# jake3991/sonar-SLAM

Hardware: AMD Instinct MI355X
Metric: keyframes/sec (CFAR+ICP) on 512x1024 sonar, 5k-pt pairs (higher is better)
Workload: dtype u8 (CFAR, integer-exact) + f32/f64-accumulate (ICP); 1 GPU; BASELINE configs[1]: 4096 keyframes/step/GPU = 1024x512 SOCA-CFAR(Ntc40,Ngc10)+gate65 -> remap+nonzero+px2m -> downsample 0.5 -> remove_outlier 1.0/5 -> 5000x5000-pt ICP (p2plane30); batch_per_gpu=4096, distinct_frames=256, screened_out_pings=0, icp_mode=p2plane30, parallelism=job farm x1, icp_prep_stream=side, batches_in_flight=1, icp_converged_jobs=4096, max_points_per_frame=17494, points_capacity=32768, full=False

## Files before the change

sonar_slam_amd/csrc/sfe_icp_sweep.h:

```cpp
#pragma once
#include "sfe_icp_common.h"

#include <algorithm>
#include <cstdlib>
#include <cstring>
#include <map>
#include <type_traits>
#include <utility>

#define SW_TCAP 8192
#define SW_NS_MAX 64
#define SW_PAD (SW_NS_MAX + 4)
#define SW_GRID_MAX 8192
#define SW_T0_NT 64
#define SW_T0_TCAP 512
#define SW_T0_GRID 512
#define SW_T1_NT 256
#define SW_T1_TCAP 2048
#define SW_T1_GRID 2048
#define SW_MG_MAX 16
#define SW_MG_WORDS 272

struct StripTab {
    int ns, len;
// ... 250 lines not shown
#else
#define SW_STAMP(k)                                                                              \
    do {                                                                                         \
        if (PROF && threadIdx.x == 0 && blockIdx.x == 0 && it == SW_STAMP_ITER)                  \
            prof[85 + (k)] = clock64();                                                          \
    } while (0)
#endif

#define SW_WATCH(cnt, bound, code)                                                               \
    if (++(cnt) > (bound)) {                                                                     \
        if (dbg)                                                                                 \
            atomicMax(dbg + (code), (int)blockIdx.x + 1);                                        \
        break;                                                                                   \
    }
#define SW_NQ 8
#define SW_NONE (-1)
#define SW_INEXACT_OF(bpos) (-2 - (bpos))
#define SW_OWN_DONE 0x80000000u
#define SW_TIED 0x40000000u
#define SW_PARTIAL 0x20000000u
#define SW_QMASK 0x1FFFFFFFu
#define SW_REC_MIN_ITER 12

struct SweepQ {
    int4 *st;
    float *d2;
    int *pos;
    int *wl[2];
    int *mid;
    int *lng;
    int *order;
    int *slot_of;
    unsigned *rec;
    float2 *ssrc;
    const int *perm;
};


struct SweepLaunchArgs {
    sfe_ctx *ctx;
    const sfe_icp_params *p;
    const SweepJob *d_jobs;
    const float2 *d_src;
    const float *d_guess9;
    const float2 *d_stgt;
    const int *d_perm;
    const float2 *d_snrm;
    const float *d_mean;
    const StripTab *d_tab;
    const int *d_grid;
    int4 *d_qst;
    int *d_qwl;
    float2 *d_qssrc;
    float *d_nn_d2;
    int *d_nn_pos;
    float *d_T9;
    int32_t *d_status, *d_iters;
    long long *d_prof;
    int *d_dbg;
    int sw_budget, sw_budget_a, sw_cache, sw_cache2;
    float sw_m, sw_kappa;
    unsigned long long *d_sync;
    sfe_icp_outliers ox;
};

template <int NT, bool PROF, bool REC>
constexpr size_t sweep_ctl_bytes()
{
    return (sizeof(SweepShared<NT, PROF, REC>) + 15) & ~(size_t)15;
}

template <int NT, int MINW, bool LDS_TGT, bool LDS_Q, bool PROF, bool REC, bool MULTI>
int sweep_launch_loop(const SweepLaunchArgs &a, int n, const int *d_ids, size_t body, int t_cap, int q_cap);

template <int NT, int TCAP, int GM, bool GTAIL = false, int KMF = 0>
int sweep_launch_prep(sfe_ctx *ctx, hipStream_t ps, const sfe_icp_params *p, int n, const SweepPrep *d_preps, const int *d_pids,
// ... 17 lines not shown
```

sonar_slam_amd/csrc/sfe_icp_sweep.hip:

```cpp
#include "sfe_icp_sweep.h"

#include <vector>

int sfe_icp_sweep_launch(sfe_ctx *ctx, const sfe_icp_params *p, const IcpCall &call, const float *d_src, const float *d_tgt,
                         const int32_t *jobs4, const float *d_guess9, int n_jobs, float *d_T9, int32_t *d_status,
                         int32_t *d_iters)
{
    std::vector<SweepPrep> preps;
    std::vector<SweepJob> jobs;
    jobs.reserve((size_t)n_jobs);
    std::vector<int> ids_tiny, ids_t0, ids_t1, ids_q, ids_lds, ids_glb, ids_multi, split_first;
    std::vector<int> pids[3];
    std::vector<int> prep_tier;
    std::vector<char> prep_need;
    std::vector<int> pids_nrm;
    std::map<std::pair<int, int>, int> seen;
    long long toff = 0, qoff = 0, koff = 0, goff = 0;
    const sfe_tuning &tu = ctx->tune;
    const bool multi_on = tu.sw_multi && !(ctx->icp_variant & 16) && !call.unsplit;
    const int strip_pts = tu.sw_strip_pts;
    const long long tiny_pairs = (p->use_diff_checker || p->max_iter < SW_REC_MIN_ITER) ? SW_TINY_PAIRS_SHORT : SW_TINY_PAIRS_LONG;
    auto is_tiny = [&](int n_src, int n_tgt) {
        return tu.sw_tiny && n_src <= SW_TINY_MAX && n_tgt <= SW_TINY_MAX && (long long)n_src * n_tgt <= tiny_pairs;
    };
// ... 120 lines not shown
        for (int r : ids_q)
            route[jobs[(size_t)r].out] = SFE_ICP_ROUTE_LDS;
        std::sort(ids_lds.begin(), ids_lds.end());
        ids_q.clear();
    }
    const int n_prep = (int)preps.size(), n_rec = (int)jobs.size();
    const int n_tiny = (int)ids_tiny.size();
    const int n_t0 = (int)ids_t0.size(), n_t1 = (int)ids_t1.size(), n_q = (int)ids_q.size(), n_lds = (int)ids_lds.size(),
              n_glb = (int)ids_glb.size(), n_multi = (int)ids_multi.size(), n_split = (int)split_first.size();
    const size_t o_jobs = (sizeof(SweepPrep) * (size_t)n_prep + 15) & ~(size_t)15;
    const size_t o_ids = (o_jobs + sizeof(SweepJob) * (size_t)n_rec + 15) & ~(size_t)15;
    const size_t o_split = o_ids + sizeof(int) * (size_t)n_rec;
    const size_t o_pids = o_split + sizeof(int) * (size_t)n_split;
    const size_t o_pnrm = o_pids + sizeof(int) * (size_t)n_prep;
    const size_t tab_bytes = o_pnrm + sizeof(int) * pids_nrm.size();
    const bool side = (ctx->icp_variant & 8) != 0;
    const SfeIcpGenPlan gen = sfe_icp_gen_begin(ctx->icp_gens, side, n_split > 0);
    if (gen.sync_first) {
        SFE_HIP(ctx, hipStreamSynchronize(ctx->stream2));
        SFE_HIP(ctx, hipStreamSynchronize(ctx->stream));
    }
    enum { G_TABLES, G_STGT, G_PERM, G_SNRM, G_MEAN, G_GKEYS, G_TAB, G_GRID, G_N };
    static const int gen_slot[2][G_N] = {{12, 14, 15, 16, 17, 24, 23, 38}, {72, 73, 74, 75, 76, 77, 78, 79}};
    static_assert(SFE_NSCRATCH == 80, "generation 1 takes the last eight slots");
    const int *gs = gen_slot[gen.g];
    char *d_tables = (char *)sfe_scratch(ctx, gs[G_TABLES], tab_bytes);
    float2 *d_stgt = (float2 *)sfe_scratch(ctx, gs[G_STGT], sizeof(float2) * (size_t)toff);
    int *d_perm = (int *)sfe_scratch(ctx, gs[G_PERM], sizeof(int) * (size_t)toff);
    float2 *d_snrm = p->minimizer == 1 ? (float2 *)sfe_scratch(ctx, gs[G_SNRM], sizeof(float2) * (size_t)toff) : nullptr;
    float *d_mean = (float *)sfe_scratch(ctx, gs[G_MEAN], sizeof(float) * 2 * (size_t)n_prep);
    unsigned long long *d_gkeys =
        (unsigned long long *)sfe_scratch(ctx, gs[G_GKEYS], sizeof(unsigned long long) * (size_t)std::max(koff, 1LL));
    int4 *d_qst = (int4 *)sfe_scratch(ctx, 19, sizeof(int4) * (size_t)qoff);
    int *d_qwl = (int *)sfe_scratch(ctx, 21, sizeof(int) * 7 * (size_t)qoff);
    float2 *d_qssrc = (float2 *)sfe_scratch(ctx, 30, sizeof(float2) * (size_t)qoff);
    StripTab *d_tab = (StripTab *)sfe_scratch(ctx, gs[G_TAB], sizeof(StripTab) * (size_t)n_prep);
    int *d_grid = (int *)sfe_scratch(ctx, gs[G_GRID], sizeof(int) * (size_t)goff);
    float *d_nn_d2 = (float *)sfe_scratch(ctx, 5, sizeof(float) * (size_t)qoff);
    int *d_nn_pos = (int *)sfe_scratch(ctx, 6, sizeof(int) * (size_t)qoff);
    if (!d_tables || !d_stgt || !d_perm || (p->minimizer == 1 && !d_snrm) || !d_mean || !d_gkeys || !d_qst || !d_qwl || !d_qssrc || !d_tab || !d_grid ||
        !d_nn_d2 || !d_nn_pos)
        return SFE_ERR_HIP;
    float2 *d_gsrc = nullptr;
    unsigned long long *d_sync = nullptr;
    const size_t sync_bytes = sizeof(unsigned long long) * 2 * SW_MG_MAX * SW_MG_WORDS * (size_t)n_sync;
    if (n_split) {
        d_gsrc = (float2 *)sfe_scratch(ctx, 46, sizeof(float2) * (size_t)qoff);
        d_sync = (unsigned long long *)sfe_scratch(ctx, 45, sync_bytes);
        if (!d_gsrc || !d_sync)
            return SFE_ERR_HIP;
    }
    SweepPrep *d_preps = (SweepPrep *)d_tables;
    SweepJob *d_jobs = (SweepJob *)(d_tables + o_jobs);
    int *d_ids = (int *)(d_tables + o_ids);
    int *d_split = (int *)(d_tables + o_split);
    int *d_pids = (int *)(d_tables + o_pids);
    hipStream_t ps = side ? ctx->stream2 : ctx->stream;
    for (int g = 0; g < 2; ++g)
        if (gen.wait[g])
            SFE_HIP(ctx, hipStreamWaitEvent(ps, ctx->ev_loop[g], 0));
    if (gen.wait_begin)
        SFE_HIP(ctx, hipStreamWaitEvent(ps, ctx->ev_loop_begin, 0));
    {
// ... 85 lines not shown
            return SFE_ERR_HIP;
        SFE_HIP(ctx, hipMemsetAsync(d_dbg, 0, sizeof(int) * 8, ctx->stream));
    }
    long long *d_prof = ctx->icp_prof ? (long long *)sfe_scratch(ctx, 20, sizeof(long long) * SFE_ICP_PROF_N) : nullptr;
    if (ctx->icp_prof && !d_prof)
        return SFE_ERR_HIP;
    if (d_prof)
        SFE_HIP(ctx, hipMemsetAsync(d_prof, 0, sizeof(long long) * SFE_ICP_PROF_N, ctx->stream));
    SFE_HIP(ctx, hipEventRecord(ctx->ev_loop_begin, ctx->stream));
    SweepLaunchArgs a;
    a.ctx = ctx;
    a.p = p;
    a.d_jobs = d_jobs;
    a.d_src = (const float2 *)d_src;
    a.d_guess9 = d_guess9;
    a.d_stgt = d_stgt;
    a.d_perm = d_perm;
    a.d_snrm = d_snrm;
    a.d_mean = d_mean;
    a.d_tab = d_tab;
    a.d_grid = d_grid;
    a.d_qst = d_qst;
    a.d_qwl = d_qwl;
    a.d_qssrc = d_qssrc;
    a.d_nn_d2 = d_nn_d2;
    a.d_nn_pos = d_nn_pos;
    a.d_T9 = d_T9;
    a.d_status = d_status;
    a.d_iters = d_iters;
    a.d_prof = d_prof;
    a.d_dbg = d_dbg;
    a.sw_budget = tu.sw_budget;
    a.sw_budget_a = tu.sw_budget_a;
    a.sw_cache = sw_cache;
    a.sw_cache2 = tu.sw_union_iters | (tu.sw_union_max << 8);
    a.sw_m = 0.01f * (float)tu.sw_recm;
    a.sw_kappa = tu.sw_reck;
    a.d_sync = d_sync;
    a.ox = call.ox;
    const bool rec_build = (sw_cache & 16) != 0 && p->max_iter >= SW_REC_MIN_ITER && !p->use_diff_checker;
    int rc = 0;
    const int *ids = d_ids;
    if (n_tiny) {
        if ((rc = sweep_launch_tiny(ctx, p, n_tiny, d_jobs, ids, d_preps, (const float2 *)d_src, (const float2 *)d_tgt, d_guess9,
                                    (const int *)d_perm, (const float2 *)d_snrm, (const float *)d_mean, (const StripTab *)d_tab, d_T9,
                                    d_status, d_iters, tiny_tmax, tiny_smax, call.ox)))
            return rc;
// ... 111 lines not shown
```

sonar_slam_amd/csrc/sfe_icp_sweep_loop.hip:

```cpp
#include "sfe_icp_sweep.h"


template <class TV>
__device__ __forceinline__ int sweep_resolve_tie(const TV &T, const StripTab &tab, const SweepQ &Q,
                                                 float px, float py, float best)
{
    int bo = 0x7FFFFFFF, bp = 0;
    const int ns = tab.ns, so = strip_of(py, tab.ylo, tab.inv_g, ns);
    int s_up = so, s_dn = so - 1;
    for (int guard = 0; guard < 2 * SW_NS_MAX + 2; ++guard) {
        const int s = next_strip(tab, ns, so, s_up, s_dn, py, best);
        if (s < 0)
            break;
        const int lo = strip_lower_bound_lane(T, tab.sbeg[s], tab.sbeg[s + 1] - 1, px);
        for (int dir = 0; dir < 2; ++dir) {
            for (int j = dir ? lo : lo - 1;; j += dir ? 1 : -1) {
                const float2 t = T[j];
                const float dx = f_add(px, -t.x), e = f_mul(dx, dx);
                if (!(e <= best))
                    break;
                const float dy = f_add(py, -t.y);
                if (f_add(e, f_mul(dy, dy)) == best) {
                    const int o = Q.perm[j - 1];
                    if (o < bo) {
                        bo = o;
                        bp = j;
                    }
                }
            }
        }
    }
    return bp;
}

template <int NT, int MINW, bool LDS_TGT, bool LDS_Q, bool PROF, bool REC, bool MULTI, bool OX>
__global__ __launch_bounds__(NT, MINW) __attribute__((amdgpu_waves_per_eu(MINW, MINW))) void icp_sweep_kernel(
    sfe_icp_params P, const SweepJob *__restrict__ jobs, const int *__restrict__ job_ids, const float2 *__restrict__ src_all,
    const float *__restrict__ guess_all, const float2 *__restrict__ stgt_all, const int *__restrict__ perm_all,
    const float2 *__restrict__ snrm_all, const float *__restrict__ mean_all, const StripTab *__restrict__ tab_all,
    const int *__restrict__ grid_all, int4 *__restrict__ q_st_all, int *__restrict__ q_wl_all, float2 *__restrict__ q_ssrc_all,
    float *__restrict__ nn_d2_all,
    int *__restrict__ nn_pos_all, float *__restrict__ T_out, int *__restrict__ status_out,
    int *__restrict__ iters_out, long long *prof, int *dbg, int sw_budget, int sw_budget_a, int sw_cache, int t_cap, int q_cap, int sort_chunk, float sw_m, float sw_kappa,
    unsigned long long *__restrict__ sync_all, int sw_cache2, sfe_icp_outliers O_arg)
{
    const sfe_icp_outliers O = OX ? O_arg : sfe_icp_outliers{};

    static_assert(LDS_TGT || !LDS_Q, "LDS_Q needs the LDS-resident target layout");
    static_assert(!MULTI || !PROF, "the profile build runs whole jobs");
    static_assert(!MULTI || !REC, "split jobs run without clearance records");
    extern __shared__ __attribute__((aligned(16))) char smem_raw[];
    using Shared = SweepShared<NT, PROF, REC>;
    Shared &S = *reinterpret_cast<Shared *>(smem_raw);

    const int jb = __builtin_amdgcn_readfirstlane(job_ids[blockIdx.x]);
    SweepJob J = jobs[jb];
    J.src_start = __builtin_amdgcn_readfirstlane(J.src_start);
    J.n_src = __builtin_amdgcn_readfirstlane(J.n_src);
    J.n_tgt = __builtin_amdgcn_readfirstlane(J.n_tgt);
    J.prep = __builtin_amdgcn_readfirstlane(J.prep);
    J.out = __builtin_amdgcn_readfirstlane(J.out);
    J.grp = __builtin_amdgcn_readfirstlane(J.grp);
    J.ngrp = __builtin_amdgcn_readfirstlane(J.ngrp);
    J.sync = __builtin_amdgcn_readfirstlane(J.sync);
// ... 13 lines not shown
    float *l_d2 = reinterpret_cast<float *>(lds_tgt + t_cap);
    short *l_pos = reinterpret_cast<short *>(l_d2 + q_cap);
    auto Pz = [&](int i) -> int {
        if constexpr (LDS_Q)
            return (int)l_pos[i];
        else
            return Q.pos[i];
    };
    auto Dz = [&](int i) -> float {
        if constexpr (LDS_Q)
            return l_d2[i];
        else
            return Q.d2[i];
    };
    auto setQ = [&](int i, float d, int pz) {
        if constexpr (LDS_Q) {
            l_d2[i] = d;
            l_pos[i] = (short)pz;
        } else {
            Q.d2[i] = d;
            Q.pos[i] = pz;
        }
    };
    Q.wl[0] = q_wl_all + 7 * J.q_off;
    Q.wl[1] = Q.wl[0] + ns;
    Q.mid = Q.wl[1] + ns;
    Q.lng = Q.mid + ns;
    Q.order = Q.lng + ns;
    Q.slot_of = Q.order + ns;
    Q.rec = reinterpret_cast<unsigned *>(Q.slot_of + ns);
    Q.ssrc = q_ssrc_all + J.q_off;
    Q.perm = perm_all + J.tgt_off;
    const float *guess = guess_all + 9 * (size_t)J.out;
    const int tid = threadIdx.x, lane = threadIdx.x & 63;
    const float mx = sw_uniform(mean_all[2 * J.prep]), my = sw_uniform(mean_all[2 * J.prep + 1]);

    if (PROF && tid == 0) {
        for (int i = 0; i < 16; ++i)
            S.prof[i] = 0;
        for (int i = 0; i < 64; ++i)
            S.prof_it[i] = 0;
        S.prof_t = clock64();
    }
    unsigned long long c_eval = 0, c_coop = 0, c_wit = 0, c_lb = 0;
    if (tid == 0) {
        S.rmax_bits = 0u;
        S.xabort = 0;
    }
    {
        const int *tsrc = reinterpret_cast<const int *>(tab_all + J.prep);
        int *tdst = reinterpret_cast<int *>(&S.tab);
        for (int i = tid; i < (int)(sizeof(StripTab) / sizeof(int)); i += NT)
            tdst[i] = tsrc[i];
    }

    float T0[9];
    {
        const float Tinv[9] = {1, 0, -mx, 0, 1, -my, 0, 0, 1};
        float g[9];
#pragma unroll
        for (int i = 0; i < 9; ++i)
            g[i] = guess[i];
        mat3_mul(Tinv, g, T0);
#pragma unroll
        for (int i = 0; i < 9; ++i)
            T0[i] = sw_uniform(T0[i]);
    }
    __syncthreads();

    typedef __attribute__((address_space(1))) unsigned long long gu64;
    unsigned xepoch = 0;
    gu64 *xsync = MULTI ? (gu64 *)(sync_all + (size_t)J.sync * (size_t)(2 * SW_MG_MAX * SW_MG_WORDS)) : nullptr;
    auto xpoll = [&](gu64 *g, unsigned epoch) -> unsigned {
        unsigned long long x = __hip_atomic_load(g, __ATOMIC_RELAXED, __HIP_MEMORY_SCOPE_AGENT);
        if ((unsigned)(x >> 32) != epoch) {
            const unsigned long long t0 = wall_clock64();
            while (true) {
                __builtin_amdgcn_s_sleep(8);
                x = __hip_atomic_load(g, __ATOMIC_RELAXED, __HIP_MEMORY_SCOPE_AGENT);
                if ((unsigned)(x >> 32) == epoch)
                    break;
                if (wall_clock64() - t0 > 50000000ull) {
                    S.xabort = 1;
                    break;
                }
            }
        }
        return (unsigned)x;
    };
    auto xbail = [&]() {
// ... 29 lines not shown
        if (tid < 20)
            __hip_atomic_store(bank + J.grp * SW_MG_WORDS + tid,
                               ((unsigned long long)xepoch << 32) | reinterpret_cast<const unsigned *>(S.acc)[tid],
                               __ATOMIC_RELAXED, __HIP_MEMORY_SCOPE_AGENT);
        double tot = 0.0;
        if (tid < 10) {
            for (int w = 0; w < J.ngrp; ++w) {
                const unsigned lo = xpoll(bank + w * SW_MG_WORDS + 2 * tid, xepoch);
                const unsigned hi = xpoll(bank + w * SW_MG_WORDS + 2 * tid + 1, xepoch);
                tot += __hiloint2double((int)hi, (int)lo);
            }
        }
        __syncthreads();
        if (tid < 10)
            S.acc[tid] = tot;
        __syncthreads();
        if (S.xabort)
            xbail();
    };
    const int *__restrict__ grid = (grid_all != nullptr && (sw_cache & 4) != 0)
                                       ? grid_all + 64 * (size_t)__builtin_amdgcn_readfirstlane(S.tab.grid_off64) : nullptr;

    {
        unsigned long long *skeys = reinterpret_cast<unsigned long long *>(lds_tgt);
        float rloc = 0.0f;
        int *scnt = reinterpret_cast<int *>(S.hist);
        auto qpos = [&](int q) {
            const float2 sp = src[q];
            return make_float2(affine1(T0[0], T0[1], T0[2], sp.x, sp.y), affine1(T0[3], T0[4], T0[5], sp.x, sp.y));
        };
        for (int c0 = 0; c0 < ns; c0 += sort_chunk) {
            const int n = min(sort_chunk, ns - c0);
            unsigned n2 = 2;
            while (n2 < (unsigned)n)
                n2 <<= 1;
            if (tid < SW_NS_MAX)
                scnt[tid] = 0;
            __syncthreads();
            for (unsigned i = tid; i < (unsigned)n; i += NT) {
                const float2 r = qpos(c0 + i);
                atomicAdd(&scnt[strip_of(r.y, S.tab.ylo, S.tab.inv_g, S.tab.ns)], 1);
                const float rr = sqrtf(f_add(f_mul(r.x, r.x), f_mul(r.y, r.y)));
                rloc = (rr > rloc || rr != rr) ? rr : rloc;
            }
            __syncthreads();
            strip_sort_lds<NT>(skeys, (unsigned)n, n2, scnt, reinterpret_cast<int *>(S.hist0), [&](unsigned i) {
                const float2 r = qpos(c0 + i);
                return SW_KEY(strip_of(r.y, S.tab.ylo, S.tab.inv_g, S.tab.ns), mono_key(r.x), c0 + i);
            });
            for (int i = tid; i < n; i += NT) {
                const int q = SW_KEY_ID(skeys[i]);
                Q.order[c0 + i] = q;
                Q.ssrc[c0 + i] = src[q];
                Q.slot_of[q] = c0 + i;
                Q.rec[c0 + i] = 0u;
            }
            __syncthreads();
        }
        atomicMax(&S.rmax_bits, __float_as_uint(rloc));
    }
    if (LDS_TGT) {
        for (int i = tid; i < nt + SW_PAD; i += NT)
            lds_tgt[i] = stgt[i];
    }
    if (tid == 0) {
        S.chk_n[0] = 1;
        S.chk_n[1] = 0;
        S.chk_n[2] = 0;
        const float I[9] = {1, 0, 0, 0, 1, 0, 0, 0, 1};
        for (int i = 0; i < 9; ++i)
            S.Ti[i] = I[i];
        S.flag_iterate = 1;
        S.flag_status = SFE_ICP_OK;
        S.hist_c[0] = 1.0f;
        S.hist_s[0] = 0.0f;
        S.hist_x[0] = 0.0f;
        S.hist_y[0] = 0.0f;
    }
// ... 12 lines not shown
    if constexpr (OX) {
        if (O.use_median && O.median_factor < 1.0f)
            Cmax = sw_uniform(r2_match);
    }
    float Cinit;
    {
        const float h = 8.0f * tab.ext_x / (float)nt;
        Cinit = h * h;
        if (!(Cinit > 1e-30f) || !(Cinit < Cmax))
            Cinit = Cmax;
        Cinit = sw_uniform(Cinit);
    }
    float Cnext = sw_uniform(P.use_trimmed_filter ? Cinit : Cmax);
    if constexpr (OX) {
        if (O.use_median)
            Cnext = sw_uniform(Cinit);
    }
    SW_PROF(0);

    const int sw_rtrips = (sw_cache >> 8) & 255;
    const bool sw_jump = (sw_cache & 2) != 0;
    const float sw_margin = sw_uniform(1.0f + 0.01f * (float)((sw_cache >> 16) & 255));
    int wd_outer = 0;
    auto xform = [&](const float (&Ti)[9], float2 sp) {
        const float rx = affine1(T0[0], T0[1], T0[2], sp.x, sp.y);
        const float ry = affine1(T0[3], T0[4], T0[5], sp.x, sp.y);
        return make_float2(affine1(Ti[0], Ti[1], Ti[2], rx, ry), affine1(Ti[3], Ti[4], Ti[5], rx, ry));
    };
    bool use_cache = false;
    const bool sw_rec = REC && (sw_cache & 16) != 0;
    const float M2 = sw_uniform(f_mul(f_add(1.0f, sw_m), f_add(1.0f, sw_m)));
    int rec_epoch = 0;
    const float rmax = sw_uniform(f_mul(__uint_as_float(S.rmax_bits), 1.00001f));
    int it = 0;
    float limit_prev = INFINITY;
    while (true) {
        SW_WATCH(wd_outer, P.max_iter + 2, 0)
        float Ti[9];
#pragma unroll
        for (int i = 0; i < 9; ++i)
            Ti[i] = sw_uniform(S.Ti[i]);
        if (sw_rec && it < ICP_MAX_HIST) {
            if (tid < it) {
                const float a0 = f_add(Ti[0], -S.thist[tid][0]), a1 = f_add(Ti[1], -S.thist[tid][1]);
                const float a3 = f_add(Ti[3], -S.thist[tid][3]), a4 = f_add(Ti[4], -S.thist[tid][4]);
                const float tx = f_add(Ti[2], -S.thist[tid][2]), ty = f_add(Ti[5], -S.thist[tid][5]);
                const float f2 = f_add(f_add(f_mul(a0, a0), f_mul(a1, a1)), f_add(f_mul(a3, a3), f_mul(a4, a4)));
                const float det = f_add(f_mul(a0, a4), -f_mul(a1, a3));
                const float disc = fmaxf(f_add(f_mul(f2, f2), -f_mul(4.0f, f_mul(det, det))), 0.0f);
                const float fa = f_mul(sqrtf(f_mul(0.5f, f_add(f2, sqrtf(disc)))), 1.001f);
// ... 153 lines not shown
                if (tid == 0) {
                    S.long_n = 0;
                    S.long_next = 0;
                    S.mid_n = 0;
                    S.wl_n[cur ^ 1] = 0;
                }
                __syncthreads();
                if (round == 0)
                    SW_STAMP(1);
                if (round == 0 && sw_rec && use_cache && it < ICP_MAX_HIST) {
                    const float mv_last = sw_uniform(f_add(f_mul(S.mva[it - 1], rmax), S.mvt[it - 1]));
                    const float mu = f_mul(sw_kappa, mv_last);
                    rec_on = mu < 0.5f * sqrtf(C);
                    mu2 = sw_uniform(f_mul(mu, mu));
                    triage = rec_on && rec_epoch < it && (rec_epoch == it - 1 || 2u * rechit_prev >= (unsigned)ns) &&
                             (sw_cache & 32) != 0;
                    predict = triage && (sw_cache & (1 << 25)) != 0 && (sw_cache & (1 << 26)) != 0 && P.use_trimmed_filter &&
                              limit_prev < INFINITY && limit_prev > 0.0f;
                }
                const bool rec_use = rec_on && rec_epoch < it;
                const int *wl = Q.wl[cur];
                int *wl_next = Q.wl[cur ^ 1];
                auto walk_pass = [&](const int *list, int n, bool fresh, int budget, bool last) {
                float2 sp_next = make_float2(0, 0);
                int q_next = 0;
                if (fresh && tid < n) {
                    sp_next = Q.ssrc[tid];
                    q_next = Q.order[tid];
                }
                const float sC = f_mul(sqrtf(C), 1.00001f);
                for (int k0 = 0; k0 < n; k0 += NT) {
                    const int slot = k0 + tid;
                    const bool valid = slot < n;
                    const float2 sp_cur = sp_next;
                    const int q_cur = q_next;
                    int prev = 0;
                    const unsigned rec = (fresh && rec_use && valid) ? Q.rec[slot] : 0u;
                    if (fresh && use_cache && valid)
                        prev = Pz(q_cur);
                    if (fresh && slot + NT < n) {
                        sp_next = Q.ssrc[slot + NT];
                        q_next = Q.order[slot + NT];
                    }
                    int q = 0, bpos = 0;
                    float px = 0, py = 0, best = W2;
                    float second = INFINITY;
                    bool tied = false, own_done = false;
                    if (valid) {
                        if (fresh) {
                            q = q_cur;
                            const float2 p = xform(Ti, sp_cur);
                            px = p.x;
                            py = p.y;
                        } else {
                            const unsigned e = (unsigned)list[slot];
                            q = (int)(e & SW_QMASK);
                            own_done = (e & SW_OWN_DONE) != 0;
                            tied = (e & SW_TIED) != 0;
                            const float2 p = xform(Ti, src[q]);
                            px = p.x;
                            py = p.y;
                            bpos = -2 - Pz(q);
                            best = Dz(q);
                            if (e & SW_PARTIAL)
                                second = __int_as_float(Q.st[q].z);
                        }
                    }
                    bool skip = false, grid_hit = false, grid_defer = false, rec_hit = false;
                    if (fresh && use_cache && valid) {
                        const int w = prev >= 0 ? prev + 1 : (prev <= -3 ? -2 - prev : 0);
                        if (PROF)
                            c_wit += (unsigned long long)__popcll(__ballot(w != 0));
                        if (w) {
                            const float2 t = T[w];
                            const float dxw = f_add(px, -t.x), dyw = f_add(py, -t.y);
                            const float dw = f_add(f_mul(dxw, dxw), f_mul(dyw, dyw));
                            if (dw < best) {
                                best = dw;
                                bpos = w;
                                if (rec != 0u && (int)(rec & 63u) >= rec_epoch && dw < r2m_up) {
                                    const float ux = f_add(px, -Ti[2]), uy = f_add(py, -Ti[5]);
                                    const float xr = f_mul(sqrtf(f_add(f_mul(ux, ux), f_mul(uy, uy))), 1.0001f);
// ... 219 lines not shown
                    if (is_none) {
                        setQ(q, INFINITY, SW_NONE);
                        if (!skip)
                            Q.st[q] = make_int4(__float_as_int(px), __float_as_int(py),
                                                __float_as_int(f_add(f_mul(sqrtf(best), 0.99999f), -md_hi)), 0);
                    }
                    if (is_exact) {
                        if (tied)
                            bpos = sweep_resolve_tie(T, tab, Q, px, py, best);
                        setQ(q, best, bpos - 1);
                    }
                    if (is_susp || is_long)
                        setQ(q, best, SW_INEXACT_OF(bpos));
                    if (rec_on && (is_exact || is_susp) && !rec_hit) {
                        unsigned r = 0u;
                        if (!grid_hit && it < ICP_MAX_HIST) {
                            const float capv = (best < r2m_up) ? C : best;
                            const float edge = f_add(f_mul(best < capv ? best : capv, M2), mu2);
                            const float R = f_mul(sqrtf(fminf(second, edge)), 0.99999f);
                            r = (__float_as_uint(R) & ~63u) | (unsigned)it;
                            if (!(R > 0.0f))
                                r = 0u;
                        }
                        Q.rec[fresh ? slot : Q.slot_of[q]] = r;
                    }
                    if (rec_on && is_long) {
                        Q.st[q].z = __float_as_int(second);
                        Q.rec[fresh ? slot : Q.slot_of[q]] = 0u;
                    }
                    tally_settled(is_none, is_exact, best);
                    if (__ballot(grid_hit || grid_defer) && lane == 0)
                        S.grid_skips = 1;
                    {
                        const unsigned long long ms = __ballot(is_susp), ml = __ballot(is_long);
                        const unsigned long long below = (1ull << lane) - 1ull;
                        if (ms) {
                            int base = 0;
                            if (lane == 0)
                                base = atomicAdd(&S.wl_n[cur ^ 1], __popcll(ms));
                            base = __builtin_amdgcn_readfirstlane(base);
                            if (is_susp)
                                wl_next[base + __popcll(ms & below)] = q;
                        }
                        if (ml) {
                            int base = 0;
                            if (lane == 0)
                                base = atomicAdd(last ? &S.long_n : &S.mid_n, __popcll(ml));
                            base = __builtin_amdgcn_readfirstlane(base);
                            if (is_long) {
                                const unsigned e = (unsigned)q | (own_fin ? SW_OWN_DONE : 0u) | (tied ? SW_TIED : 0u) |
                                                   ((rec_on && !last) ? SW_PARTIAL : 0u);
                                (last ? Q.lng : Q.mid)[base + __popcll(ml & below)] = (int)e;
                            }
                        }
                    }
                }
                };
                auto triage_pass = [&]() {
                    const float sC = f_mul(sqrtf(C), 1.00001f);
                    int *wl_next = Q.wl[cur ^ 1];
                    int q_n = 0;
                    float2 sp_n = make_float2(0, 0);
                    unsigned rec_n = 0u;
                    if (tid < ns) {
                        q_n = Q.order[tid];
                        sp_n = Q.ssrc[tid];
                        rec_n = Q.rec[tid];
                    }
                    for (int k0 = 0; k0 < ns; k0 += NT) {
                        const int slot = k0 + tid;
                        const bool valid = slot < ns;
                        int q = 0, bpos = 0;
                        float px = 0, py = 0, best = W2;
                        bool skip = false, rec_hit = false;
                        const int q_c = q_n;
                        const float2 sp = sp_n;
                        const unsigned rec = rec_n;
                        if (slot + NT < ns) {
                            q_n = Q.order[slot + NT];
                            sp_n = Q.ssrc[slot + NT];
                            rec_n = Q.rec[slot + NT];
                        }
                        if (valid) {
                            q = q_c;
                            const int prev = Pz(q);
                            const float2 p = xform(Ti, sp);
                            px = p.x;
                            py = p.y;
                            const int w = prev >= 0 ? prev + 1 : (prev <= -3 ? -2 - prev : 0);
                            if (w) {
                                const float2 t = T[w];
                                const float dxw = f_add(px, -t.x), dyw = f_add(py, -t.y);
                                const float dw = f_add(f_mul(dxw, dxw), f_mul(dyw, dyw));
                                if (dw < best) {
                                    best = dw;
                                    bpos = w;
                                    if (rec != 0u && (int)(rec & 63u) >= rec_epoch && dw < r2m_up) {
                                        const float ux = f_add(px, -Ti[2]), uy = f_add(py, -Ti[5]);
                                        const float xr = f_mul(sqrtf(f_add(f_mul(ux, ux), f_mul(uy, uy))), 1.0001f);
                                        const float mv = f_add(f_mul(S.mva[rec & 63u], xr), S.mvt[rec & 63u]);
                                        const float Ro = f_add(__uint_as_float(rec & ~63u), -mv);
                                        rec_hit = f_mul(sqrtf(dw), 1.00001f) < Ro || (dw > C && sC < Ro);
                                    }
                                }
                            } else if (prev == SW_NONE) {
// ... 7 lines not shown
                            const unsigned long long mh = __ballot(rec_hit);
                            if (mh && lane == 0)
                                atomicAdd(&S.n_rechit[it & 1], (unsigned)__popcll(mh));
                        }
                        const bool lane_done = !valid || skip || rec_hit || !(px == px && py == py);
                        const bool is_long = valid && !lane_done;
                        const bool settled = valid && lane_done;
                        const bool found = best < r2m_up;
                        const bool is_none = settled && !found;
                        const bool is_exact = settled && found && best <= C;
                        const bool is_susp = settled && found && !(best <= C);
                        if (is_none) {
                            setQ(q, INFINITY, SW_NONE);
                            if (!skip)
                                Q.st[q] = make_int4(__float_as_int(px), __float_as_int(py),
                                                    __float_as_int(f_add(f_mul(sqrtf(best), 0.99999f), -md_hi)), 0);
                        }
                        if (is_exact)
                            setQ(q, best, bpos - 1);
                        if (is_susp || is_long)
                            setQ(q, best, SW_INEXACT_OF(bpos));
                        if (is_long) {
                            Q.st[q].z = __float_as_int(INFINITY);
                            Q.rec[slot] = 0u;
                        }
                        tally_settled(is_none, is_exact, best, !predict);
                        const unsigned long long ms = __ballot(is_susp), ml = __ballot(is_long);
                        const unsigned long long below = (1ull << lane) - 1ull;
                        if (ms) {
                            int base = 0;
                            if (lane == 0)
                                base = atomicAdd(&S.wl_n[cur ^ 1], __popcll(ms));
                            base = __builtin_amdgcn_readfirstlane(base);
                            if (is_susp)
                                wl_next[base + __popcll(ms & below)] = q;
                        }
                        if (ml) {
                            int base = 0;
                            if (lane == 0)
                                base = atomicAdd(&S.mid_n, __popcll(ml));
                            base = __builtin_amdgcn_readfirstlane(base);
                            if (is_long)
                                Q.mid[base + __popcll(ml & below)] = (int)((unsigned)q | SW_PARTIAL);
                        }
                    }
                };
                if (round == 0) {
// ... 12 lines not shown
                }
                __syncthreads();
                SW_PROF(6);
                SW_STAMP(3);
                const int nlong = S.long_n;
                if (PROF && tid == 0) {
                    S.prof[SW_PI(9)] += 1;
                    S.prof[SW_PI(10)] += nlong;
                }
                if (nlong > 0) {
                    const bool left = lane < 32;
                    auto next_slot = [&]() {
                        int v = 0;
                        if (lane == 0)
                            v = atomicAdd(&S.long_next, 1);
                        return __builtin_amdgcn_readfirstlane(v);
                    };
                    int slot = next_slot();
                    int qn = 0, posn = 0;
                    float2 pn = make_float2(0, 0);
                    float bn = 0;
                    auto fetch = [&](int sl) {
                        qn = (int)((unsigned)Q.lng[sl] & SW_QMASK);
                        pn = src[qn];
                        bn = Dz(qn);
                        posn = Pz(qn);
                    };
                    if (slot < nlong)
                        fetch(slot);
                    int wd2 = 0;
                    while (slot < nlong) {
                        SW_WATCH(wd2, ns + 2, 5)
                        long long tp0 = 0;
                        if (PROF && tid == 0)
                            tp0 = clock64();
                        const int q = __builtin_amdgcn_readfirstlane(qn);
                        const float2 pq = xform(Ti, make_float2(sw_uniform(pn.x), sw_uniform(pn.y)));
                        const float px = sw_uniform(pq.x), py = sw_uniform(pq.y);
                        float best = sw_uniform(bn);
                        int bpos = -2 - __builtin_amdgcn_readfirstlane(posn);
                        bool tied = false;
                        slot = next_slot();
                        if (slot < nlong)
                            fetch(slot);
                        if (PROF && tid == 0) {
                            const long long t_ = clock64();
                            S.prof[SW_PI(13)] += t_ - tp0;
// ... 325 lines not shown
            auto kept = [&](int i, bool in, int &id, unsigned &cnt) -> bool {
                float d = 0.0f;
                id = -1;
                if (in) {
                    id = Pz(i);
                    d = Dz(i);
                }
                bool ok = in && id >= 0 && (!P.use_max_dist_filter || d <= r2_filter) &&
                          (!P.use_trimmed_filter || d <= limit);
                if constexpr (OX)
                    ok = ok && icp_ox_keep(O, min2, med_limit, d);
                cnt += (unsigned)__popcll(__ballot(ok));
                return ok;
            };
            const int roles = min(SW_SUM_ROLES, (ns + 63) >> 6);
            for (int w0 = tid >> 6; w0 < roles; w0 += NT / 64) {
                double a[NA] = {0, 0, 0, 0, 0, 0, 0, 0, 0};
                unsigned cnt = 0;
                if (P.minimizer == 0) {
                    for (int base = 64 * w0; base < ns; base += 1024) {
                        const int i = base + lane;
                        int id;
                        if (kept(i, i < ns, id, cnt)) {
                            const float2 p = xform(Ti, src[i]);
                            const float2 q = T[id + 1];
                            const double px = p.x, py = p.y, qx = q.x, qy = q.y;
                            a[0] += px;
                            a[1] += py;
                            a[2] += qx;
                            a[3] += qy;
                            a[4] += qx * px;
                            a[5] += qx * py;
                            a[6] += qy * px;
                            a[7] += qy * py;
                        }
                    }
                } else {
                    for (int base = 64 * w0; base < ns; base += 1024) {
                        const int i = base + lane;
                        int id;
                        if (kept(i, i < ns, id, cnt)) {
                            const float2 sp = src[i];
                            const float2 n = snrm[id];
                            const float2 q = T[id + 1];
                            const float2 p = xform(Ti, sp);
                            const double px = p.x, py = p.y, nx = n.x, ny = n.y;
                            const double a0 = px * ny - py * nx;
                            const double e = nx * (px - (double)q.x) + ny * (py - (double)q.y);
                            a[0] += a0 * a0;
                            a[1] += a0 * nx;
                            a[2] += a0 * ny;
                            a[3] += nx * nx;
                            a[4] += nx * ny;
                            a[5] += ny * ny;
                            a[6] += -(a0 * e);
                            a[7] += -(nx * e);
                            a[8] += -(ny * e);
                        }
                    }
                }
                static_assert(NA == WSP_N + 1, "the plan's accumulators");
                const double sk = wave_sum_n(a);
                S.red[NA * w0 + wsp_final_slot(lane & 15)] = sk;
                if (lane == 0)
                    S.xr[w0] = cnt;
// ... 27 lines not shown
            icp_solve_and_check<OX>(P, O, acc, Ti, S.Ti, chk, status, iterate);
            S.chk_n[0] = chk.nhist;
            S.chk_n[1] = chk.counter;
            S.chk_n[2] = chk.iters;
            S.flag_status = status;
            S.flag_iterate = (status == SFE_ICP_OK) ? iterate : 0;
        }
        __syncthreads();
        SW_PROF(5);
        SW_STAMP(8);
        if (!S.flag_iterate)
            break;
        use_cache = (sw_cache & 1) != 0;
        if (!rec_on)
            rec_epoch = it + 1;
        ++it;
    }

    if (tid == 0 && (!MULTI || J.grp == 0)) {
        const int status = S.flag_status;
        float *To = T_out + 9 * (size_t)J.out;
        if (status == SFE_ICP_OK) {
            const float Tfwd[9] = {1, 0, mx, 0, 1, my, 0, 0, 1};
            float Ti[9], tmp[9], res[9];
            for (int i = 0; i < 9; ++i)
                Ti[i] = S.Ti[i];
            mat3_mul(Ti, T0, tmp);
            mat3_mul(Tfwd, tmp, res);
            for (int i = 0; i < 9; ++i)
                To[i] = res[i];
        } else {
            for (int i = 0; i < 9; ++i)
                To[i] = guess[i];
        }
        status_out[J.out] = status;
        iters_out[J.out] = S.chk_n[2];
        if (PROF && blockIdx.x == 0) {
            for (int i = 0; i < 16; ++i)
                prof[i] = S.prof[i];
            for (int i = 0; i < 64; ++i)
                prof[16 + i] = S.prof_it[i];
        }
    }
    if (PROF && lane == 0) {
        atomicAdd((unsigned long long *)&prof[80], c_eval);
        atomicAdd((unsigned long long *)&prof[81], c_coop);
        atomicAdd((unsigned long long *)&prof[82], c_wit);
        atomicAdd((unsigned long long *)&prof[83], c_lb);
        if (tid == 0)
// ... 94 lines not shown
        jobs[j0 + tid].n_src = (tid < G) ? s_goff[g + 1] - s_goff[g] : 0;
        jobs[j0 + tid].q_off = J.q_off + s_goff[g];
    }
}

static int pow2_floor(size_t v)
{
    size_t p = 1;
    while (2 * p <= v)
        p *= 2;
    return (int)p;
}

template <int NT, int MINW, bool LDS_TGT, bool LDS_Q, bool PROF, bool REC, bool MULTI>
int sweep_launch_loop(const SweepLaunchArgs &a, int n, const int *d_ids, size_t body, int t_cap, int q_cap)
{
    sfe_ctx *ctx = a.ctx;
    const sfe_icp_outliers &ox = a.ox;
    auto kernel = (ox.use_min_dist || ox.use_median || ox.use_bound) ? icp_sweep_kernel<NT, MINW, LDS_TGT, LDS_Q, PROF, REC, MULTI, true>
                                                                     : icp_sweep_kernel<NT, MINW, LDS_TGT, LDS_Q, PROF, REC, MULTI, false>;
    const size_t smem = sweep_ctl_bytes<NT, PROF, REC>() + body;
    SFE_HIP(ctx, hipFuncSetAttribute((const void *)kernel, hipFuncAttributeMaxDynamicSharedMemorySize, (int)smem));
    hipLaunchKernelGGL(kernel, dim3(n), dim3(NT), smem, ctx->stream, *a.p, a.d_jobs, d_ids, a.d_src, a.d_guess9, a.d_stgt,
                       a.d_perm, a.d_snrm, a.d_mean, a.d_tab, a.d_grid, a.d_qst, a.d_qwl, a.d_qssrc, a.d_nn_d2, a.d_nn_pos,
                       a.d_T9, a.d_status, a.d_iters, a.d_prof, a.d_dbg, a.sw_budget, a.sw_budget_a, a.sw_cache, t_cap, q_cap,
                       pow2_floor(body / 8), a.sw_m, a.sw_kappa, a.d_sync, a.sw_cache2, ox);
    SFE_LAUNCH_CHECK(ctx);
    return 0;
}

#define SW_LOOP_INST(...) template int sweep_launch_loop<__VA_ARGS__>(const SweepLaunchArgs &, int, const int *, size_t, int, int);
#ifdef SW_INSPECT
SW_LOOP_INST(ICP_THREADS, 8, true, true, false, true, false)
#else
SW_LOOP_INST(SW_T0_NT, 4, true, true, false, true, false)
SW_LOOP_INST(SW_T0_NT, 4, true, true, false, false, false)
SW_LOOP_INST(SW_T1_NT, 4, true, true, true, false, false)
SW_LOOP_INST(SW_T1_NT, 4, true, true, false, true, false)
SW_LOOP_INST(SW_T1_NT, 4, true, true, false, false, false)
SW_LOOP_INST(ICP_THREADS, 4, true, true, false, false, false)
SW_LOOP_INST(ICP_THREADS, 8, true, true, true, true, false)
SW_LOOP_INST(ICP_THREADS, 8, true, true, true, false, false)
SW_LOOP_INST(ICP_THREADS, 8, true, true, false, true, false)
SW_LOOP_INST(ICP_THREADS, 8, true, true, false, false, false)
SW_LOOP_INST(ICP_THREADS, 4, true, false, false, false, false)
SW_LOOP_INST(ICP_THREADS, 8, true, false, true, false, false)
SW_LOOP_INST(ICP_THREADS, 8, true, false, false, true, false)
SW_LOOP_INST(ICP_THREADS, 8, true, false, false, false, false)
// ... 29 lines not shown
```

sonar_slam_amd/csrc/sfe_internal.h:

```cpp
#pragma once
#include <hip/hip_runtime.h>

#include <cstdarg>
#include <cstdio>
#include <string>
#include <vector>

#include "../../include/sonarfe.h"
#include "sfe_icp_gen.h"

#define SFE_NSCRATCH 80
#define SFE_ICP_PROF_N 96

struct sfe_tuning {
    int cfar_os_gated = 1;
    int cfar_os_gated_min = 40;
    int cfar_os_pref = 1;
    int cfar_os_pref_x = 80;
    int extract_rec_cap = 0;
    int extract_capw = 0;
    int extract_compact = 1;
    int cost_many = 1;
    int sw_tiers = 1;
    int sw_tiny = 1;
    int sw_multi = 1;
    int sw_multi_g = 0;
    int sw_multi_min_src = 8192;
    int sw_multi_share_min = 1024;
    int sw_cache = 1;
    int sw_rec = 1;
    int sw_budget = 128;
    int sw_budget_a = 6;
    int sw_margin = 15;
    int sw_rtrips = 4;
// ... 163 lines not shown
```

Measured before the change: 167,700 keyframes/s.

## Pack sweep slot data into 16-byte records and cache pre-transformed sources

Merges the per-slot order index, rec word and sorted source point into one aligned 16-byte SweepSlot record, so the walk and triage passes fetch each slot with a single vector load instead of three separate loads. Source points are also stored already transformed by the initial guess T0 (rsrc), so xform applies only the current increment, dropping one affine transform per point lookup. T0 is now rebuilt at the end instead of being held in registers for the whole loop. The cost is an extra scratch buffer and partial 4-byte writes into the 16-byte records when rec is updated.

```diff
diff --git a/sonar_slam_amd/csrc/sfe_icp_sweep.h b/sonar_slam_amd/csrc/sfe_icp_sweep.h
--- a/sonar_slam_amd/csrc/sfe_icp_sweep.h
+++ b/sonar_slam_amd/csrc/sfe_icp_sweep.h
@@ -296,6 +296,13 @@
 #define SW_QMASK 0x1FFFFFFFu
 #define SW_REC_MIN_ITER 12
 
+struct __attribute__((aligned(16))) SweepSlot {
+    float rx, ry;
+    int order;
+    unsigned rec;
+};
+static_assert(sizeof(SweepSlot) == 16, "one 16-byte load per slot");
+
 struct SweepQ {
     int4 *st;
     float *d2;
@@ -303,10 +310,9 @@
     int *wl[2];
     int *mid;
     int *lng;
-    int *order;
+    SweepSlot *slot;
     int *slot_of;
-    unsigned *rec;
-    float2 *ssrc;
+    float2 *rsrc;
     const int *perm;
 };
 
@@ -325,7 +331,8 @@
     const int *d_grid;
     int4 *d_qst;
     int *d_qwl;
-    float2 *d_qssrc;
+    float2 *d_qrsrc;
+    SweepSlot *d_qslot;
     float *d_nn_d2;
     int *d_nn_pos;
     float *d_T9;
diff --git a/sonar_slam_amd/csrc/sfe_icp_sweep.hip b/sonar_slam_amd/csrc/sfe_icp_sweep.hip
--- a/sonar_slam_amd/csrc/sfe_icp_sweep.hip
+++ b/sonar_slam_amd/csrc/sfe_icp_sweep.hip
@@ -166,7 +166,7 @@
     }
     enum { G_TABLES, G_STGT, G_PERM, G_SNRM, G_MEAN, G_GKEYS, G_TAB, G_GRID, G_N };
     static const int gen_slot[2][G_N] = {{12, 14, 15, 16, 17, 24, 23, 38}, {72, 73, 74, 75, 76, 77, 78, 79}};
-    static_assert(SFE_NSCRATCH == 80, "generation 1 takes the last eight slots");
+    static_assert(SFE_NSCRATCH == 81, "generation 1 takes slots 72..79, the loop kernel's slot records the last one");
     const int *gs = gen_slot[gen.g];
     char *d_tables = (char *)sfe_scratch(ctx, gs[G_TABLES], tab_bytes);
     float2 *d_stgt = (float2 *)sfe_scratch(ctx, gs[G_STGT], sizeof(float2) * (size_t)toff);
@@ -176,13 +176,14 @@
     unsigned long long *d_gkeys =
         (unsigned long long *)sfe_scratch(ctx, gs[G_GKEYS], sizeof(unsigned long long) * (size_t)std::max(koff, 1LL));
     int4 *d_qst = (int4 *)sfe_scratch(ctx, 19, sizeof(int4) * (size_t)qoff);
-    int *d_qwl = (int *)sfe_scratch(ctx, 21, sizeof(int) * 7 * (size_t)qoff);
-    float2 *d_qssrc = (float2 *)sfe_scratch(ctx, 30, sizeof(float2) * (size_t)qoff);
+    int *d_qwl = (int *)sfe_scratch(ctx, 21, sizeof(int) * 5 * (size_t)qoff);
+    float2 *d_qrsrc = (float2 *)sfe_scratch(ctx, 30, sizeof(float2) * (size_t)qoff);
+    SweepSlot *d_qslot = (SweepSlot *)sfe_scratch(ctx, 80, sizeof(SweepSlot) * (size_t)qoff);
     StripTab *d_tab = (StripTab *)sfe_scratch(ctx, gs[G_TAB], sizeof(StripTab) * (size_t)n_prep);
     int *d_grid = (int *)sfe_scratch(ctx, gs[G_GRID], sizeof(int) * (size_t)goff);
     float *d_nn_d2 = (float *)sfe_scratch(ctx, 5, sizeof(float) * (size_t)qoff);
     int *d_nn_pos = (int *)sfe_scratch(ctx, 6, sizeof(int) * (size_t)qoff);
-    if (!d_tables || !d_stgt || !d_perm || (p->minimizer == 1 && !d_snrm) || !d_mean || !d_gkeys || !d_qst || !d_qwl || !d_qssrc || !d_tab || !d_grid ||
+    if (!d_tables || !d_stgt || !d_perm || (p->minimizer == 1 && !d_snrm) || !d_mean || !d_gkeys || !d_qst || !d_qwl || !d_qrsrc || !d_qslot || !d_tab || !d_grid ||
         !d_nn_d2 || !d_nn_pos)
         return SFE_ERR_HIP;
     float2 *d_gsrc = nullptr;
@@ -314,7 +315,8 @@
     a.d_grid = d_grid;
     a.d_qst = d_qst;
     a.d_qwl = d_qwl;
-    a.d_qssrc = d_qssrc;
+    a.d_qrsrc = d_qrsrc;
+    a.d_qslot = d_qslot;
     a.d_nn_d2 = d_nn_d2;
     a.d_nn_pos = d_nn_pos;
     a.d_T9 = d_T9;
diff --git a/sonar_slam_amd/csrc/sfe_icp_sweep_loop.hip b/sonar_slam_amd/csrc/sfe_icp_sweep_loop.hip
--- a/sonar_slam_amd/csrc/sfe_icp_sweep_loop.hip
+++ b/sonar_slam_amd/csrc/sfe_icp_sweep_loop.hip
@@ -38,8 +38,8 @@
     sfe_icp_params P, const SweepJob *__restrict__ jobs, const int *__restrict__ job_ids, const float2 *__restrict__ src_all,
     const float *__restrict__ guess_all, const float2 *__restrict__ stgt_all, const int *__restrict__ perm_all,
     const float2 *__restrict__ snrm_all, const float *__restrict__ mean_all, const StripTab *__restrict__ tab_all,
-    const int *__restrict__ grid_all, int4 *__restrict__ q_st_all, int *__restrict__ q_wl_all, float2 *__restrict__ q_ssrc_all,
-    float *__restrict__ nn_d2_all,
+    const int *__restrict__ grid_all, int4 *__restrict__ q_st_all, int *__restrict__ q_wl_all, float2 *__restrict__ q_rsrc_all,
+    SweepSlot *__restrict__ q_slot_all, float *__restrict__ nn_d2_all,
     int *__restrict__ nn_pos_all, float *__restrict__ T_out, int *__restrict__ status_out,
     int *__restrict__ iters_out, long long *prof, int *dbg, int sw_budget, int sw_budget_a, int sw_cache, int t_cap, int q_cap, int sort_chunk, float sw_m, float sw_kappa,
     unsigned long long *__restrict__ sync_all, int sw_cache2, sfe_icp_outliers O_arg)
@@ -99,14 +99,13 @@
             Q.pos[i] = pz;
         }
     };
-    Q.wl[0] = q_wl_all + 7 * J.q_off;
+    Q.wl[0] = q_wl_all + 5 * J.q_off;
     Q.wl[1] = Q.wl[0] + ns;
     Q.mid = Q.wl[1] + ns;
     Q.lng = Q.mid + ns;
-    Q.order = Q.lng + ns;
-    Q.slot_of = Q.order + ns;
-    Q.rec = reinterpret_cast<unsigned *>(Q.slot_of + ns);
-    Q.ssrc = q_ssrc_all + J.q_off;
+    Q.slot_of = Q.lng + ns;
+    Q.slot = q_slot_all + J.q_off;
+    Q.rsrc = q_rsrc_all + J.q_off;
     Q.perm = perm_all + J.tgt_off;
     const float *guess = guess_all + 9 * (size_t)J.out;
     const int tid = threadIdx.x, lane = threadIdx.x & 63;
@@ -131,8 +130,7 @@
             tdst[i] = tsrc[i];
     }
 
-    float T0[9];
-    {
+    auto make_T0 = [&](float (&T0)[9]) {
         const float Tinv[9] = {1, 0, -mx, 0, 1, -my, 0, 0, 1};
         float g[9];
 #pragma unroll
@@ -142,7 +140,7 @@
 #pragma unroll
         for (int i = 0; i < 9; ++i)
             T0[i] = sw_uniform(T0[i]);
-    }
+    };
     __syncthreads();
 
     typedef __attribute__((address_space(1))) unsigned long long gu64;
@@ -218,6 +216,8 @@
                                        ? grid_all + 64 * (size_t)__builtin_amdgcn_readfirstlane(S.tab.grid_off64) : nullptr;
 
     {
+        float T0[9];
+        make_T0(T0);
         unsigned long long *skeys = reinterpret_cast<unsigned long long *>(lds_tgt);
         float rloc = 0.0f;
         int *scnt = reinterpret_cast<int *>(S.hist);
@@ -246,10 +246,15 @@
             });
             for (int i = tid; i < n; i += NT) {
                 const int q = SW_KEY_ID(skeys[i]);
-                Q.order[c0 + i] = q;
-                Q.ssrc[c0 + i] = src[q];
+                const float2 r = qpos(q);
+                SweepSlot sl;
+                sl.rx = r.x;
+                sl.ry = r.y;
+                sl.order = q;
+                sl.rec = 0u;
+                Q.slot[c0 + i] = sl;
+                Q.rsrc[q] = r;
                 Q.slot_of[q] = c0 + i;
-                Q.rec[c0 + i] = 0u;
             }
             __syncthreads();
         }
@@ -308,10 +313,8 @@
     const bool sw_jump = (sw_cache & 2) != 0;
     const float sw_margin = sw_uniform(1.0f + 0.01f * (float)((sw_cache >> 16) & 255));
     int wd_outer = 0;
-    auto xform = [&](const float (&Ti)[9], float2 sp) {
-        const float rx = affine1(T0[0], T0[1], T0[2], sp.x, sp.y);
-        const float ry = affine1(T0[3], T0[4], T0[5], sp.x, sp.y);
-        return make_float2(affine1(Ti[0], Ti[1], Ti[2], rx, ry), affine1(Ti[3], Ti[4], Ti[5], rx, ry));
+    auto xform = [&](const float (&Ti)[9], float2 r) {
+        return make_float2(affine1(Ti[0], Ti[1], Ti[2], r.x, r.y), affine1(Ti[3], Ti[4], Ti[5], r.x, r.y));
     };
     bool use_cache = false;
     const bool sw_rec = REC && (sw_cache & 16) != 0;
@@ -511,26 +514,21 @@
                 const int *wl = Q.wl[cur];
                 int *wl_next = Q.wl[cur ^ 1];
                 auto walk_pass = [&](const int *list, int n, bool fresh, int budget, bool last) {
-                float2 sp_next = make_float2(0, 0);
-                int q_next = 0;
-                if (fresh && tid < n) {
-                    sp_next = Q.ssrc[tid];
-                    q_next = Q.order[tid];
-                }
+                SweepSlot sl_next = {0.0f, 0.0f, 0, 0u};
+                if (fresh && tid < n)
+                    sl_next = Q.slot[tid];
                 const float sC = f_mul(sqrtf(C), 1.00001f);
                 for (int k0 = 0; k0 < n; k0 += NT) {
                     const int slot = k0 + tid;
                     const bool valid = slot < n;
-                    const float2 sp_cur = sp_next;
-                    const int q_cur = q_next;
+                    const float2 sp_cur = make_float2(sl_next.rx, sl_next.ry);
+                    const int q_cur = sl_next.order;
                     int prev = 0;
-                    const unsigned rec = (fresh && rec_use && valid) ? Q.rec[slot] : 0u;
+                    const unsigned rec = (fresh && rec_use && valid) ? sl_next.rec : 0u;
                     if (fresh && use_cache && valid)
                         prev = Pz(q_cur);
-                    if (fresh && slot + NT < n) {
-                        sp_next = Q.ssrc[slot + NT];
-                        q_next = Q.order[slot + NT];
-                    }
+                    if (fresh && slot + NT < n)
+                        sl_next = Q.slot[slot + NT];
                     int q = 0, bpos = 0;
                     float px = 0, py = 0, best = W2;
                     float second = INFINITY;
@@ -546,7 +544,7 @@
                             q = (int)(e & SW_QMASK);
                             own_done = (e & SW_OWN_DONE) != 0;
                             tied = (e & SW_TIED) != 0;
-                            const float2 p = xform(Ti, src[q]);
+                            const float2 p = xform(Ti, Q.rsrc[q]);
                             px = p.x;
                             py = p.y;
                             bpos = -2 - Pz(q);
@@ -812,11 +810,11 @@
                             if (!(R > 0.0f))
                                 r = 0u;
                         }
-                        Q.rec[fresh ? slot : Q.slot_of[q]] = r;
+                        Q.slot[fresh ? slot : Q.slot_of[q]].rec = r;
                     }
                     if (rec_on && is_long) {
                         Q.st[q].z = __float_as_int(second);
-                        Q.rec[fresh ? slot : Q.slot_of[q]] = 0u;
+                        Q.slot[fresh ? slot : Q.slot_of[q]].rec = 0u;
                     }
                     tally_settled(is_none, is_exact, best);
                     if (__ballot(grid_hit || grid_defer) && lane == 0)
@@ -849,28 +847,20 @@
                 auto triage_pass = [&]() {
                     const float sC = f_mul(sqrtf(C), 1.00001f);
                     int *wl_next = Q.wl[cur ^ 1];
-                    int q_n = 0;
-                    float2 sp_n = make_float2(0, 0);
-                    unsigned rec_n = 0u;
-                    if (tid < ns) {
-                        q_n = Q.order[tid];
-                        sp_n = Q.ssrc[tid];
-                        rec_n = Q.rec[tid];
-                    }
+                    SweepSlot sl_n = {0.0f, 0.0f, 0, 0u};
+                    if (tid < ns)
+                        sl_n = Q.slot[tid];
                     for (int k0 = 0; k0 < ns; k0 += NT) {
                         const int slot = k0 + tid;
                         const bool valid = slot < ns;
                         int q = 0, bpos = 0;
                         float px = 0, py = 0, best = W2;
                         bool skip = false, rec_hit = false;
-                        const int q_c = q_n;
-                        const float2 sp = sp_n;
-                        const unsigned rec = rec_n;
-                        if (slot + NT < ns) {
-                            q_n = Q.order[slot + NT];
-                            sp_n = Q.ssrc[slot + NT];
-                            rec_n = Q.rec[slot + NT];
-                        }
+                        const int q_c = sl_n.order;
+                        const float2 sp = make_float2(sl_n.rx, sl_n.ry);
+                        const unsigned rec = sl_n.rec;
+                        if (slot + NT < ns)
+                            sl_n = Q.slot[slot + NT];
                         if (valid) {
                             q = q_c;
                             const int prev = Pz(q);
@@ -924,7 +914,7 @@
                             setQ(q, best, SW_INEXACT_OF(bpos));
                         if (is_long) {
                             Q.st[q].z = __float_as_int(INFINITY);
-                            Q.rec[slot] = 0u;
+                            Q.slot[slot].rec = 0u;
                         }
                         tally_settled(is_none, is_exact, best, !predict);
                         const unsigned long long ms = __ballot(is_susp), ml = __ballot(is_long);
@@ -983,7 +973,7 @@
                     float bn = 0;
                     auto fetch = [&](int sl) {
                         qn = (int)((unsigned)Q.lng[sl] & SW_QMASK);
-                        pn = src[qn];
+                        pn = Q.rsrc[qn];
                         bn = Dz(qn);
                         posn = Pz(qn);
                     };
@@ -1355,7 +1345,7 @@
                         const int i = base + lane;
                         int id;
                         if (kept(i, i < ns, id, cnt)) {
-                            const float2 p = xform(Ti, src[i]);
+                            const float2 p = xform(Ti, Q.rsrc[i]);
                             const float2 q = T[id + 1];
                             const double px = p.x, py = p.y, qx = q.x, qy = q.y;
                             a[0] += px;
@@ -1373,7 +1363,7 @@
                         const int i = base + lane;
                         int id;
                         if (kept(i, i < ns, id, cnt)) {
-                            const float2 sp = src[i];
+                            const float2 sp = Q.rsrc[i];
                             const float2 n = snrm[id];
                             const float2 q = T[id + 1];
                             const float2 p = xform(Ti, sp);
@@ -1447,9 +1437,10 @@
         float *To = T_out + 9 * (size_t)J.out;
         if (status == SFE_ICP_OK) {
             const float Tfwd[9] = {1, 0, mx, 0, 1, my, 0, 0, 1};
-            float Ti[9], tmp[9], res[9];
+            float Ti[9], T0[9], tmp[9], res[9];
             for (int i = 0; i < 9; ++i)
                 Ti[i] = S.Ti[i];
+            make_T0(T0);
             mat3_mul(Ti, T0, tmp);
             mat3_mul(Tfwd, tmp, res);
             for (int i = 0; i < 9; ++i)
@@ -1590,8 +1581,8 @@
     const size_t smem = sweep_ctl_bytes<NT, PROF, REC>() + body;
     SFE_HIP(ctx, hipFuncSetAttribute((const void *)kernel, hipFuncAttributeMaxDynamicSharedMemorySize, (int)smem));
     hipLaunchKernelGGL(kernel, dim3(n), dim3(NT), smem, ctx->stream, *a.p, a.d_jobs, d_ids, a.d_src, a.d_guess9, a.d_stgt,
-                       a.d_perm, a.d_snrm, a.d_mean, a.d_tab, a.d_grid, a.d_qst, a.d_qwl, a.d_qssrc, a.d_nn_d2, a.d_nn_pos,
-                       a.d_T9, a.d_status, a.d_iters, a.d_prof, a.d_dbg, a.sw_budget, a.sw_budget_a, a.sw_cache, t_cap, q_cap,
+                       a.d_perm, a.d_snrm, a.d_mean, a.d_tab, a.d_grid, a.d_qst, a.d_qwl, a.d_qrsrc, a.d_qslot, a.d_nn_d2,
+                       a.d_nn_pos, a.d_T9, a.d_status, a.d_iters, a.d_prof, a.d_dbg, a.sw_budget, a.sw_budget_a, a.sw_cache, t_cap, q_cap,
                        pow2_floor(body / 8), a.sw_m, a.sw_kappa, a.d_sync, a.sw_cache2, ox);
     SFE_LAUNCH_CHECK(ctx);
     return 0;
diff --git a/sonar_slam_amd/csrc/sfe_internal.h b/sonar_slam_amd/csrc/sfe_internal.h
--- a/sonar_slam_amd/csrc/sfe_internal.h
+++ b/sonar_slam_amd/csrc/sfe_internal.h
@@ -9,7 +9,7 @@
 #include "../../include/sonarfe.h"
 #include "sfe_icp_gen.h"
 
-#define SFE_NSCRATCH 80
+#define SFE_NSCRATCH 81
 #define SFE_ICP_PROF_N 96
 
 struct sfe_tuning {
```

After: 172,000 keyframes/s, median of 6. +2.5%, better.
